# Rose-STL-Lab/dyffusion

Hardware: AMD Instinct MI355X
Metric: sampled fields/sec (h-step rollout) (higher is better)
Workload: dtype bf16; 1 GPU; BASELINE configs[1]: Navier-Stokes 221x42, C=3+2 static ch, unet_simple dim 64 @256^2, DYffusion h=16 cold sampling + refine, interpolator MC dropout p=0.15, hipGraph rollout; rows_per_gpu=80, total_rows=80, net_forwards_per_rollout=60, parallelism=ensemble-sharded dp1

## Files before the change

dyffusion_amd/csrc/engine.hip:

```cpp
#include "engine_internal.h"

#include <dlfcn.h>
#include <mutex>
#include <rccl/rccl.h>
#include "unet_kernels.h"
#include "../../include/dyffusion_hip_testing.h"

using namespace dyf;

namespace {

thread_local bool g_creating_group_child = false;

int default_row_groups(const dyf_engine* e) {
    if (e->cfg.net[0].arch != DYF_ARCH_UNET_RESNET || e->cfg.net[1].arch != DYF_ARCH_UNET_RESNET) return 1;
    if (e->cfg.batch_invariant) return 1;
    const long long plane = (long long)e->cfg.height * e->cfg.width;
    if (plane > 128 * 128) return 1;
    const long long pix = plane * e->cfg.max_batch;
    if (pix >= 72ll * 60 * 60) return 3;
    return 1;
}

void layout_blocks(Net& n) {
// ... 217 lines not shown
        if (f.up_cols) sparse_out = &b;
        const bool prof = e->prof_layer == i && e->prof_ev.size() < 4096;
        hipEvent_t pe0 = nullptr, pe1 = nullptr;
        if (prof) {
            HIP_TRY(e, hipEventCreate(&pe0));
            HIP_TRY(e, hipEventCreate(&pe1));
        }
        const bool commute = dyf_form_int("DYF_DEC_COMMUTE", 1) != 0;
        const bool commuted = commute && b.k == 1 && b.stride == 1 && b.pad == 0 && e->cfg.enable_mfma && (b.cout & 3) == 0 &&
                              (size_t)nb * lh * lw * b.cout * sizeof(float) <= (size_t)nb * b.in_h * b.in_w * b.cin * sizeof(el16_t);
        if (use_fused_up(e, b, f)) {
            if (prof) HIP_TRY(e, hipEventRecord(pe0, st));
            HIP_TRY(e, launch_conv(f, b.wpk, 1, st));
            if (prof) HIP_TRY(e, hipEventRecord(pe1, st));
        } else if (commuted) {
            ConvArgs lo = a;
            lo.src0 = x; lo.c0 = b.cin - skip_c; lo.src1 = skip; lo.c1 = skip_c;
            lo.h = lh; lo.w = lw; lo.ho = lh; lo.wo = lw;
            lo.coef_a = ws.ones_f; lo.coef_c = ws.zeros_f; lo.coef_stride = 0; lo.coef_div = 0;
            lo.act = ACT_NONE; lo.drop = DropSpec{};
            lo.out_el16 = nullptr; lo.out_f32 = (float*)ws.up;
            if (prof) HIP_TRY(e, hipEventRecord(pe0, st));
            dyf_status s = run_conv(e, lo, b.wpk, st);
            if (s != DYF_OK) return s;
            Up2xEpiArgs u{};
            u.lo = (const float*)ws.up; u.n = nb; u.h = lh; u.w = lw; u.c = b.cout;
            u.coef_a = a.coef_a; u.coef_c = a.coef_c; u.coef_stride = a.coef_stride; u.coef_div = a.coef_div;
            u.act = a.act; u.drop = a.drop; u.out = a.out_el16;
            HIP_TRY(e, launch_up2x_epilogue(u, st));
            if (prof) HIP_TRY(e, hipEventRecord(pe1, st));
        } else {
            Up2xArgs u{};
            u.src0 = x; u.c0 = b.cin - skip_c; u.src1 = skip; u.c1 = skip_c; u.n = nb; u.h = lh; u.w = lw; u.out = ws.up;
            HIP_TRY(e, launch_up2x(u, st));
            a.src0 = ws.up; a.c0 = b.cin; a.src1 = nullptr; a.c1 = 0;
            if (prof) HIP_TRY(e, hipEventRecord(pe0, st));
            dyf_status s = run_conv(e, a, b.wpk, st);
            if (s != DYF_OK) return s;
            if (prof) HIP_TRY(e, hipEventRecord(pe1, st));
        }
        if (prof) {
            e->prof_ev.emplace_back(pe0, pe1);
            e->prof_rows.push_back(nb);
        }
        x = ws.dec[i - 6];
        lh = b.out_h; lw = b.out_w;
        if (i < 11) {
            skip = ws.enc[10 - i];
            skip_c = n.blk[10 - i].cout;
        }
    }
    ReadoutArgs r{};
    r.x = x; r.n = nb; r.ih = lh; r.iw = lw; r.cin = n.dim; r.wgt = n.ro_w; r.wfrag = n.ro_wfrag; r.bias = n.ro_b; r.cout = n.cfg.out_channels;
    r.oh = H; r.ow = W; r.out = out_dev; r.nearest = n.cfg.outer_nearest;
    e->last_dec5_sparse = sparse_out != nullptr;
    r.iw_store = sparse_out ? sparse_out->up_wo_store : lw;
    r.col_map = sparse_out ? sparse_out->up_col_map : nullptr;
    if (n.ro_row_tab && (sparse_out != nullptr) == n.ro_tab_sparse) {
        r.row_tab = n.ro_row_tab;
        r.col_tab = n.ro_col_tab;
    }
    HIP_TRY(e, launch_readout(r, st));
    return DYF_OK;
}

dyf_status compute_coefs(dyf_engine* e, Net& n, const float* time_dev, int rows, float* coef_a, float* coef_c,
                         hipStream_t st) {
    FilmArgs f{};
    if (n.cfg.with_time_emb) {
        TimeMlpArgs t{};
        t.time = time_dev; t.rows = rows; t.dim = n.dim; t.w1 = n.t_w1; t.b1 = n.t_b1; t.w2 = n.t_w2; t.b2 = n.t_b2;
        t.silu_out = e->ws.silu;
        if (n.t_learned) { t.learned_w = n.t_learned; t.learned_half = n.cfg.learned_sinusoidal_dim / 2; }
        HIP_TRY(e, launch_time_mlp(t, st));
        f.silu = e->ws.silu;
    }
    f.rows = rows; f.tdim = n.tdim; f.total_c = n.total_c; f.wf = n.film_w; f.bf = n.film_b; f.blk_of = n.blk_of;
    f.blk_off = n.blk_off; f.blk_cout = n.blk_cout; f.norm_a = n.norm_a; f.norm_c = n.norm_c; f.coef_a = coef_a;
    f.coef_c = coef_c;
    HIP_TRY(e, launch_film(f, st));
    return DYF_OK;
}

}

extern "C" {

int32_t dyf_abi_version(void) { return DYF_ABI_VERSION; }

int32_t dyf_dtype(void) { return DYF_F16 ? DYF_DTYPE_F16 : DYF_DTYPE_BF16; }

const char* dyf_last_error(const dyf_engine* engine) { return engine ? engine->err.c_str() : g_create_error.c_str(); }

static void destroy_groups(dyf_engine* e) {
    for (dyf_engine* c : e->groups) {
        if (c->group_stream) { (void)hipStreamSynchronize(c->group_stream); (void)hipStreamDestroy(c->group_stream); }
        if (c->group_done) (void)hipEventDestroy(c->group_done);
        dyf_engine_destroy(c);
    }
    e->groups.clear();
    e->last_groups = 0;
}

static void traj_release(dyf_engine* e);

void dyf_engine_destroy(dyf_engine* e) {
    if (!e) return;
    (void)hipSetDevice(e->cfg.device);
    destroy_groups(e);
    if (e->group_fork) (void)hipEventDestroy(e->group_fork);
    for (auto& kv : e->graphs) {
        if (kv.second.exec) (void)hipGraphExecDestroy(kv.second.exec);
        if (kv.second.graph) (void)hipGraphDestroy(kv.second.graph);
    }
    rn_destroy(e->net[0]);
    rn_destroy(e->net[1]);
    sc_destroy(e->net[0]);
    sc_destroy(e->net[1]);
    (void)dyf_comm_destroy(e);
    if (e->s_log) (void)hipFree(e->s_log);
    if (e->cap_stream) (void)hipStreamDestroy(e->cap_stream);
    if (e->gn_err_host) (void)hipHostFree(e->gn_err_host);
    traj_release(e);
    f32_destroy(e);
    train_destroy(e);
    release_allocs(e->allocs);
    release_allocs(e->net_allocs[0]);
    release_allocs(e->net_allocs[1]);
    release_allocs(e->plan_allocs);
    delete e;
}

dyf_status dyf_engine_create(const dyf_engine_config* cfg, dyf_engine** out_engine) {
    if (!cfg || !out_engine) return fail(nullptr, DYF_ERR_INVALID_ARGUMENT, "null argument");
    if (cfg->abi_version != DYF_ABI_VERSION) return fail(nullptr, DYF_ERR_INVALID_ARGUMENT, "ABI version mismatch");
    if (cfg->dtype != dyf_dtype())
        return fail(nullptr, DYF_ERR_INVALID_ARGUMENT, std::string("this library is the ") + DYF_DTYPE_NAME +
                    " build: engine dtype must match (libdyffusion_hip.so = bf16, libdyffusion_hip_f16.so = fp16)");
    if (cfg->height < 1 || cfg->width < 1 || cfg->max_batch < 1)
        return fail(nullptr, DYF_ERR_INVALID_ARGUMENT, "height, width and max_batch must be positive");
    int ndev = 0;
    if (hipGetDeviceCount(&ndev) != hipSuccess || ndev < 1)
        return fail(nullptr, DYF_ERR_HIP, "no HIP device available: the DYffusion engine requires an MI355X (gfx950)");
    if (cfg->device < 0 || cfg->device >= ndev) return fail(nullptr, DYF_ERR_INVALID_ARGUMENT, "device ordinal out of range");
    if (hipSetDevice(cfg->device) != hipSuccess) return fail(nullptr, DYF_ERR_HIP, "hipSetDevice failed");

    dyf_engine* e = new dyf_engine();
    e->cfg = *cfg;
    e->fuse_up2x = dyf_form_int("DYF_FUSE_UP2X", e->fuse_up2x) != 0;
    e->fuse_min_plane = (int)dyf_form_int("DYF_FUSE_MIN_PLANE", e->fuse_min_plane);
    e->fuse_stem = dyf_form_int("DYF_FUSE_STEM", e->fuse_stem) != 0;
    e->pair_interp = dyf_form_int("DYF_PAIR_INTERP", e->pair_interp) != 0;
    e->poison_dec5 = dyf_form_int("DYF_POISON_DEC5", e->poison_dec5) != 0;
    if (conv_init() != hipSuccess || linattn_fused_init() != hipSuccess || hipStreamCreateWithFlags(&e->cap_stream, hipStreamNonBlocking) != hipSuccess) {
        delete e;
        return fail(nullptr, DYF_ERR_HIP, "engine initialisation failed (conv_init / stream create)");
    }
    auto bail = [&](dyf_status st, const std::string& m) {
        g_create_error = m;
        dyf_engine_destroy(e);
        return st;
    };
    for (int w = 0; w < 2; ++w) {
        Net& n = e->net[w];
        n.cfg = cfg->net[w];
        if (n.cfg.arch != DYF_ARCH_UNET_SIMPLE && n.cfg.arch != DYF_ARCH_UNET_RESNET && n.cfg.arch != DYF_ARCH_SIMPLE_CONV_NET)
            return bail(DYF_ERR_UNSUPPORTED, "arch must be unet_simple (0), unet / resnet (1) or simple_conv_net (2)");
        if (n.cfg.dim < 4 || (n.cfg.dim & 1)) return bail(DYF_ERR_INVALID_ARGUMENT, "dim must be even and >= 4");
        if (n.cfg.input_dropout < 0.0f || n.cfg.input_dropout >= 1.0f) return bail(DYF_ERR_INVALID_ARGUMENT, "input_dropout must be in [0, 1)");
        if (n.cfg.input_dropout != 0.0f && n.cfg.arch == DYF_ARCH_SIMPLE_CONV_NET)
            return bail(DYF_ERR_UNSUPPORTED, "input_dropout > 0: arch simple_conv_net has no such layer");
        if (n.cfg.dropout < 0.0f || n.cfg.dropout >= 1.0f) return bail(DYF_ERR_INVALID_ARGUMENT, "dropout must be in [0, 1)");
        n.cin_total = n.cfg.in_channels + n.cfg.cond_channels;
        if (n.cin_total < 1 || n.cin_total > DYF_MAX_IN_CH || n.cfg.out_channels < 1 || n.cfg.out_channels > DYF_MAX_OUT_CH)
            return bail(DYF_ERR_UNSUPPORTED, "channel counts outside the supported range (inputs+cond <= 32, outputs <= 8)");
        n.dim = n.cfg.dim;
        n.tdim = 2 * n.cfg.dim;
        if (n.cfg.arch == DYF_ARCH_UNET_RESNET) {
            if (n.cfg.block_dropout1 < 0.0f || n.cfg.block_dropout1 >= 1.0f || n.cfg.attn_dropout < 0.0f || n.cfg.attn_dropout >= 1.0f)
                return bail(DYF_ERR_INVALID_ARGUMENT, "dropout rates must be in [0, 1)");
            std::string m = rn_configure(e, n);
            if (!m.empty()) return bail(DYF_ERR_INVALID_ARGUMENT, m);
            continue;
        }
        if (n.cfg.arch == DYF_ARCH_SIMPLE_CONV_NET) {
            std::string m = sc_configure(e, n);
            if (!m.empty()) return bail(DYF_ERR_INVALID_ARGUMENT, m);
            continue;
        }
        n.n_drop_sites = (n.cfg.dropout > 0.0f ? 12 : 0) + (n.cfg.input_dropout > 0.0f ? 1 : 0);
        layout_blocks(n);
        std::string m = layout_geometry(n, cfg->height, cfg->width);
        if (!m.empty()) return bail(DYF_ERR_INVALID_ARGUMENT, m);
    }
    const size_t nb = (size_t)cfg->max_batch * 2;
    size_t stem_el = 0, enc_el[6] = {}, dec_el[6] = {}, up_el = 0, raw_el = 0, tc = 0, td = 0, ub_el = 0;
    for (int w = 0; w < 2; ++w) {
        const Net& n = e->net[w];
        stem_el = std::max(stem_el, nb * n.uh * n.uw * n.dim);
        for (int i = 0; i < 6; ++i) {
            const UBlock& b = n.blk[i];
            enc_el[i] = std::max(enc_el[i], nb * b.out_h * b.out_w * b.cout);
            const UBlock& d = n.blk[6 + i];
            dec_el[i] = std::max(dec_el[i], nb * d.out_h * d.out_w * d.cout);
            up_el = std::max(up_el, nb * d.in_h * d.in_w * d.cin);
            ub_el = std::max(ub_el, conv_up_border_floats((int)nb, d.out_h / 2, d.out_w / 2, d.cout));
        }
        raw_el = std::max(raw_el, nb * n.blk[5].out_h * n.blk[5].out_w * n.blk[5].cout);
        tc = std::max<size_t>(tc, n.total_c);
        td = std::max<size_t>(td, n.tdim);
    }
    Workspace& ws = e->ws;
#define ALLOC(ptr, count)                                           \
    do {                                                            \
        dyf_status _s = dev_alloc(e, &(ptr), (count));              \
        if (_s != DYF_OK) return bail(_s, e->err);                  \
    } while (0)
    ALLOC(ws.stem, stem_el);
    {
        size_t s16 = 0;
        for (int w = 0; w < 2; ++w) s16 = std::max(s16, nb * (size_t)(e->net[w].uh + 2) * (e->net[w].uw + 2) * 16);
        ALLOC(ws.stem16, s16);
    }
    for (int i = 0; i < 6; ++i) {
        ALLOC(ws.enc[i], enc_el[i]);
        ALLOC(ws.dec[i], dec_el[i]);
    }
    ALLOC(ws.enc5_raw, raw_el);
    ALLOC(ws.up, up_el);
    ALLOC(ws.silu, nb * td);
    ALLOC(ws.coef_a, nb * tc);
    ALLOC(ws.coef_c, nb * tc);
    ALLOC(ws.zero_page, 256);
    ALLOC(ws.up_border, ub_el);
    ALLOC(ws.coef_pair, 4 * tc);
    ALLOC(ws.splitk, DYF_SPLITK_FLOATS);
    {
        size_t cmax = 64;
        for (int w = 0; w < 2; ++w)
            for (int i = 0; i < 12; ++i) cmax = std::max<size_t>(cmax, (size_t)e->net[w].blk[i].cout);
        ALLOC(ws.zeros_f, cmax);
        ALLOC(ws.ones_f, cmax);
        std::vector<float> ones(cmax, 1.0f);
        if (hipMemcpy(ws.ones_f, ones.data(), cmax * sizeof(float), hipMemcpyHostToDevice) != hipSuccess)
            return bail(DYF_ERR_HIP, "hipMemcpy(ones)");
    }
    ALLOC(e->s_pair, 2 * (size_t)cfg->max_batch * DYF_MAX_OUT_CH * cfg->height * cfg->width);
    ALLOC(e->s_time, 64);
    ALLOC(e->rng_state, DYF_RNG_STATE_WORDS);
    ALLOC(e->row_keys, 4 * nb);
#undef ALLOC
    if (hipHostMalloc((void**)&e->gn_err_host, 64, hipHostMallocMapped) == hipSuccess) {
        memset(e->gn_err_host, 0, 64);
        if (hipHostGetDevicePointer((void**)&e->gn_err_dev, e->gn_err_host, 0) != hipSuccess) e->gn_err_dev = nullptr;
    }
    if (!e->gn_err_dev) e->gn_fuse_disabled = true;
    if (dyf_form_int("DYF_GN_FUSED", 1) == 0) e->gn_fuse_disabled = true;
    {
        dyf_status rs = rn_alloc_workspace(e);
        if (rs != DYF_OK) return bail(rs, e->err);
        rs = sc_alloc_workspace(e);
        if (rs != DYF_OK) return bail(rs, e->err);
    }
    e->group_min_rows = (int)std::max(1LL, dyf_form_int("DYF_GROUP_MIN_ROWS", e->group_min_rows));
    *out_engine = e;
    if (!g_creating_group_child) {
        const int g = (int)dyf_form_int("DYF_ROW_GROUPS", default_row_groups(e));
        if (g > 1) {
            dyf_status gs = dyf_set_row_groups(e, g);
            if (gs != DYF_OK) {
                g_create_error = e->err;
                dyf_engine_destroy(e);
                *out_engine = nullptr;
                return gs;
            }
        }
    }
    return DYF_OK;
}

dyf_status dyf_set_row_groups(dyf_engine* e, int32_t n_groups) {
    if (!e) return DYF_ERR_INVALID_ARGUMENT;
    if (e->is_group_child) return fail(e, DYF_ERR_STATE, "row groups do not nest");
    if (n_groups < 1 || n_groups > 8) return fail(e, DYF_ERR_INVALID_ARGUMENT, "n_groups must be in [1, 8]");
    if (e->net[0].loaded || e->net[1].loaded)
        return fail(e, DYF_ERR_STATE, "dyf_set_row_groups must be called before dyf_load_weights (the groups hold their own packed weights)");
    HIP_TRY(e, hipSetDevice(e->cfg.device));
    HIP_TRY(e, hipDeviceSynchronize());
    destroy_groups(e);
    if (n_groups == 1 || e->cfg.max_batch < 2 * e->group_min_rows) return DYF_OK;
    n_groups = std::min<int>(n_groups, e->cfg.max_batch / e->group_min_rows);
    if (!e->group_fork) HIP_TRY(e, hipEventCreateWithFlags(&e->group_fork, hipEventDisableTiming));
    dyf_engine_config cc = e->cfg;
    cc.max_batch = (e->cfg.max_batch + std::min(n_groups, 2) - 1) / std::min(n_groups, 2);
    for (int g = 0; g < n_groups; ++g) {
        dyf_engine* c = nullptr;
        g_creating_group_child = true;
        dyf_status cs = dyf_engine_create(&cc, &c);
        g_creating_group_child = false;
        if (cs != DYF_OK) {
            destroy_groups(e);
            return fail(e, cs, "row group engine: " + g_create_error);
        }
        c->is_group_child = true;
        c->attn_dropout_exact = e->attn_dropout_exact;
        c->form_rows_scale = dyf_form_int("DYF_GROUP_FORM_SCALE", 1) != 0 ? n_groups : 1;
        e->groups.push_back(c);
// ... 1943 lines not shown
```

dyffusion_amd/csrc/kernels.h:

```cpp
#pragma once
#include "common.h"

#include <vector>

#define DYF_MAX_IN_CH 32
#define DYF_MAX_OUT_CH 8

struct TimeMlpArgs {
    const float* time;
    int rows, dim;
    const float* w1;
    const float* b1;
    const float* w2;
    const float* b2;
    float* silu_out;
    const float* learned_w = nullptr;
    int learned_half = 0;
};
hipError_t launch_time_mlp(const TimeMlpArgs& a, hipStream_t s);

struct FilmArgs {
    const float* silu;
    int rows, tdim, total_c;
    const float* wf;
    const float* bf;
    const int* blk_of;
    const int* blk_off;
    const int* blk_cout;
    const float* norm_a;
    const float* norm_c;
    float* coef_a;
    float* coef_c;
};
hipError_t launch_film(const FilmArgs& a, hipStream_t s);

struct StemArgs {
    const float* src[4];
    int ch[4];
    int nsrc, cin;
    int n, h, w;
    int src_rows;
    int out_pitch;
    int distinct_only;
    int uh, uw;
    int resample;
    int nearest;
    const float* wgt;
    const float* bias;
    int dim;
    el16_t* out;
    DropSpec drop;
    uint32_t* rng_state;
    uint32_t* rng_row_keys;
    int rng_rows, rng_rows_per_fwd;
};
hipError_t launch_stem(const StemArgs& a, hipStream_t s);
hipError_t launch_stem16(const StemArgs& a, hipStream_t s);
inline __host__ __device__ int stem16_out_rows(const StemArgs& a) { return a.distinct_only && a.src_rows > 0 ? a.src_rows : a.n; }

struct Up2xArgs {
    const el16_t* src0;
    const el16_t* src1;
    int c0, c1;
    int n, h, w;
    el16_t* out;
};
hipError_t launch_up2x(const Up2xArgs& a, hipStream_t s);

struct Up2xEpiArgs {
    const float* lo;
    int n, h, w, c;
    const float* coef_a;
    const float* coef_c;
    int coef_stride, coef_div;
    int act;
    DropSpec drop;
    el16_t* out;
};
hipError_t launch_up2x_epilogue(const Up2xEpiArgs& a, hipStream_t s);

struct GroupNormArgs {
    const float* x;
    int n, hw, c, groups;
    const float* gamma;
    const float* beta;
    const float* film_a;
    const float* film_c;
    int film_stride;
    int film_div;
    int act;
    DropSpec drop;
    el16_t* out;
};
hipError_t launch_groupnorm(const GroupNormArgs& a, hipStream_t s);

struct ReadoutArgs {
    const el16_t* x;
    int n, ih, iw, cin;
    int iw_store;
    const int16_t* col_map;
    const float* wgt;
    const el16_t* wfrag;
    const float* bias;
    int cout;
    int oh, ow;
    int nearest;
    float* out;
    const uint4* row_tab;
    const uint4* col_tab;
};
hipError_t launch_readout(const ReadoutArgs& a, hipStream_t s);
hipError_t launch_readout_tables(const ReadoutArgs& a, hipStream_t s);
inline std::vector<float> pack_readout_weights(const float* w, int cin, int cout) {
    std::vector<float> pk((size_t)16 * cin * cout);
    for (int ci = 0; ci < cin; ++ci)
        for (int co = 0; co < cout; ++co)
            for (int t = 0; t < 16; ++t) pk[((size_t)t * cin + ci) * cout + co] = w[((size_t)ci * cout + co) * 16 + t];
    return pk;
}
inline std::vector<el16_t> pack_readout_frag(const std::vector<float>& pk, int cout) {
    std::vector<el16_t> wf((size_t)16 * 2 * 64 * 8, 0);
    for (int t = 0; t < 16; ++t)
        for (int h2 = 0; h2 < 2; ++h2)
            for (int lane = 0; lane < 64; ++lane) {
                const int m = lane & 15, kg = lane >> 4;
                for (int el = 0; el < 8; ++el)
                    if (m < cout)
                        wf[(((size_t)t * 2 + h2) * 64 + lane) * 8 + el] = f32_to_el16(pk[((size_t)t * 64 + h2 * 32 + kg * 8 + el) * cout + m]);
            }
    return wf;
}

hipError_t launch_cold_update(float* x_s, const float* x_cur, const float* x_next, long long count, hipStream_t s, float* copy = nullptr);
hipError_t launch_noisy_condition(float* out, const float* cond, const float* noise, float tau, long long count,
                                  int row_elems, uint32_t* rng_state, hipStream_t s);
#define DYF_RNG_STATE_WORDS 8

struct BcArgs {
    float* preds;
    int kind;
    int n_fields, rows, c, h, w, n_meta;
    const int* row_meta;
    const float* time_factor;
    int times_per_meta;
    const uint8_t* fixed_mask;
    const float* in_velocity;
    const float* vertex_y;
    const float* boundary;
};
hipError_t launch_boundary_conditions(const BcArgs& a, hipStream_t s);
hipError_t launch_nhwc_to_nchw_f32(const el16_t* src, int n, int h, int w, int w_store, int c, const int16_t* col_map,
                                   float* out, hipStream_t s);
hipError_t launch_rng_clone(uint32_t* dst, const uint32_t* src, uint32_t row_add, bool counters_only, hipStream_t s);
hipError_t launch_rng_begin_forward(uint32_t* rng_state, uint32_t* row_keys, int rows, int rows_per_fwd, hipStream_t s);
hipError_t launch_fill_f32(float* p, float v, long long count, hipStream_t s);
hipError_t launch_criterion_sum(const float* p, const float* t, long long count, int kind, double* sum, hipStream_t s);
constexpr int CRITERION_MAX_BLOCKS = 2048;
hipError_t launch_criterion_sum_det(const float* p, const float* t, long long count, int kind, double* partials, double* sum, hipStream_t s);
hipError_t launch_ensemble_metrics(const float* preds, const float* targets, int n_members, long long n_points, double* sums,
                                   hipStream_t s);
long long trajectory_metrics_blocks(int n_members, long long n_points);
hipError_t launch_trajectory_metrics(const float* const* preds_tab, const float* const* targets_tab, int n_segments, int n_members,
                                     long long n_points, long long member_stride, double* partials, double* out, double* accum,
                                     hipStream_t s);

hipError_t launch_gather_unpack(const float* recv, float* out, int world, int slots, int nb, int total_rows, long long row, hipStream_t s);
```

dyffusion_amd/csrc/kernels.hip:

```cpp
#include "kernels.h"

#include <cstdlib>

__device__ __forceinline__ float wave_sum(float v) {
#pragma unroll
    for (int off = 32; off > 0; off >>= 1) v += __shfl_xor(v, off, 64);
    return v;
}

__device__ __forceinline__ float block_sum(float v, float* scratch ) {
    v = wave_sum(v);
    const int lane = threadIdx.x & 63, wave = threadIdx.x >> 6, nw = (blockDim.x + 63) >> 6;
    __syncthreads();
    if (lane == 0) scratch[wave] = v;
    __syncthreads();
    float t = 0.0f;
    for (int i = 0; i < nw; ++i) t += scratch[i];
    return t;
}

__global__ void time_mlp_kernel(TimeMlpArgs a) {
    extern __shared__ float sh[];
    const int row = blockIdx.x, tdim = 2 * a.dim, half = a.dim / 2;
    const int dim = a.learned_w ? 2 * a.learned_half + 1 : a.dim;
// ... 1002 lines not shown
    }
#endif
}

__global__ void readout_tables_kernel(ReadoutArgs a, uint4* row_tab, uint4* col_tab) {
    const int t = blockIdx.x * blockDim.x + threadIdx.x;
    const int th = 2 * a.ih, tw = 2 * a.iw;
    if (t < a.oh) {
        int u0, u1;
        float lu;
        bilinear_coord(t, (float)th / (float)a.oh, th, u0, u1, lu, a.nearest != 0);
        int off[4];
        float w[4];
        for (int k = 0; k < 4; ++k) {
            const int par = (k + 1) & 1;
            w[k] = ((u0 & 1) == par ? 1.0f - lu : 0.0f) + ((u1 & 1) == par ? lu : 0.0f);
            const int u = (u1 & 1) == par ? u1 : u0;
            const int i = ((u + 1) >> 1) - (k >> 1);
            off[k] = (unsigned)i < (unsigned)a.ih ? i * a.iw_store * 128 : -1;
        }
        row_tab[2 * t] = make_uint4((unsigned)off[0], (unsigned)off[1], (unsigned)off[2], (unsigned)off[3]);
        row_tab[2 * t + 1] = make_uint4(__float_as_uint(w[0]), __float_as_uint(w[1]), __float_as_uint(w[2]), __float_as_uint(w[3]));
    }
    if (t < a.ow) {
        int v0, v1;
        float lv;
        bilinear_coord(t, (float)tw / (float)a.ow, tw, v0, v1, lv, a.nearest != 0);
        int off[4];
        float w[4];
        for (int k = 0; k < 4; ++k) {
            const int par = (k + 1) & 1;
            w[k] = ((v0 & 1) == par ? 1.0f - lv : 0.0f) + ((v1 & 1) == par ? lv : 0.0f);
            const int v = (v1 & 1) == par ? v1 : v0;
            const int j = ((v + 1) >> 1) - (k >> 1);
            int js = (unsigned)j < (unsigned)a.iw ? j : -1;
            if (js >= 0 && a.col_map) js = a.col_map[js];
            off[k] = js >= 0 ? js * 128 : -1;
        }
        col_tab[2 * t] = make_uint4((unsigned)off[0], (unsigned)off[1], (unsigned)off[2], (unsigned)off[3]);
        col_tab[2 * t + 1] = make_uint4(__float_as_uint(w[0]), __float_as_uint(w[1]), __float_as_uint(w[2]), __float_as_uint(w[3]));
    }
}

hipError_t launch_readout_tables(const ReadoutArgs& a, hipStream_t s) {
    const int n = a.oh > a.ow ? a.oh : a.ow;
    hipLaunchKernelGGL(readout_tables_kernel, dim3((n + 255) / 256), dim3(256), 0, s, a, (uint4*)a.row_tab, (uint4*)a.col_tab);
    return hipGetLastError();
}

__global__ __launch_bounds__(256, 4) void readout_dma_kernel(ReadoutArgs a, int groups_per_wave) {
#if defined(__HIP_DEVICE_COMPILE__)
    extern __shared__ __attribute__((aligned(16))) char rd_smem[];
    for (int i = threadIdx.x; i < 16 * 2 * 4 * 4; i += 256) {
        const int m = i & 3, kg = (i >> 2) & 3, th = i >> 4;
        ((uint4*)rd_smem)[i] = ((const uint4*)a.wfrag)[th * 64 + kg * 16 + m];
    }
    __syncthreads();
    const int lane = threadIdx.x & 63, wave = threadIdx.x >> 6;
    const int wave_id = (int)((blockIdx.x * 256 + threadIdx.x) >> 6);
    const int p = lane & 15, kg = lane >> 4;
    char* stage = rd_smem + 8192 + wave * 8192;
    const uint4* wl = (const uint4*)rd_smem + kg * 4 + (p & 3);
    const bool wrow = p < 4;
    const int total = a.n * a.oh * a.ow;
    const int th = 2 * a.ih, tw = 2 * a.iw;
    const float sh = (float)th / (float)a.oh, sw = (float)tw / (float)a.ow;
    const int plane = a.oh * a.ow;
    const size_t xbytes = (size_t)a.n * a.ih * a.iw_store * 64 * sizeof(el16_t);
    const auto rsrc = __builtin_amdgcn_make_buffer_rsrc((void*)a.x, 0, (int)(unsigned)xbytes, 0x00020000);
    const int lp = lane >> 2, lc = lane & 3;
    const unsigned piece_off = (unsigned)((lc ^ (lp & 3)) * 16);
    const int src4 = lp * 4;
    const unsigned rd_off = (unsigned)((p * 4 + (kg ^ (p & 3))) * 16);
    for (int g = 0; g < groups_per_wave; ++g) {
        const int idx0 = (wave_id * groups_per_wave + g) * 16;
        if (idx0 >= total) break;
        int idx = idx0 + p;
        const bool live = idx < total;
        if (!live) idx = total - 1;
        const int n = idx / plane;
        const int rem = idx - n * plane;
        const int oy = rem / a.ow, ox = rem - oy * a.ow;
        const uint4 rto = a.row_tab[2 * oy], rtw = a.row_tab[2 * oy + 1], cto = a.col_tab[2 * ox], ctw = a.col_tab[2 * ox + 1];
        const int nbase = n * a.ih * a.iw_store * 128;
        const int rto_[4] = {(int)rto.x, (int)rto.y, (int)rto.z, (int)rto.w};
        const int ro[4] = {rto_[0] >= 0 ? nbase + rto_[0] : -1, rto_[1] >= 0 ? nbase + rto_[1] : -1, rto_[2] >= 0 ? nbase + rto_[2] : -1,
                           rto_[3] >= 0 ? nbase + rto_[3] : -1};
        const int co_[4] = {(int)cto.x, (int)cto.y, (int)cto.z, (int)cto.w};
        const float rw[4] = {__uint_as_float(rtw.x), __uint_as_float(rtw.y), __uint_as_float(rtw.z), __uint_as_float(rtw.w)};
        const float cw[4] = {__uint_as_float(ctw.x), __uint_as_float(ctw.y), __uint_as_float(ctw.z), __uint_as_float(ctw.w)};
        int l_ro[4], l_co[4];
#pragma unroll
        for (int k = 0; k < 4; ++k) {
            l_ro[k] = __builtin_amdgcn_ds_bpermute(src4, ro[k]);
            l_co[k] = __builtin_amdgcn_ds_bpermute(src4, co_[k]);
        }
        float out[4] = {0.0f, 0.0f, 0.0f, 0.0f};
        auto issue = [&](int bt) {
            const int kh = bt >> 1;
            char* st = stage + (bt & 1) * 4096;
#pragma unroll
            for (int t = 0; t < 2; ++t) {
                const int kw = (bt & 1) * 2 + t;
                const bool ok = l_ro[kh] >= 0 && l_co[kw] >= 0;
                const unsigned vo = ok ? (unsigned)(l_ro[kh] + l_co[kw]) + piece_off : 0xFFFFFFFFu;
                __builtin_amdgcn_raw_ptr_buffer_load_lds(rsrc, (__attribute__((address_space(3))) void*)(st + (t * 2 + 0) * 1024), 16, vo, 0, 0, 0);
                __builtin_amdgcn_raw_ptr_buffer_load_lds(rsrc, (__attribute__((address_space(3))) void*)(st + (t * 2 + 1) * 1024), 16,
                                                         ok ? vo + 64u : 0xFFFFFFFFu, 0, 0, 0);
            }
        };
        asm volatile("s_waitcnt lgkmcnt(0)" ::: "memory");
        issue(0);
#pragma unroll
        for (int bt = 0; bt < 8; ++bt) {
            if (bt + 1 < 8) {
                asm volatile("s_waitcnt lgkmcnt(0)" ::: "memory");
                issue(bt + 1);
                asm volatile("s_waitcnt vmcnt(4)" ::: "memory");
            } else {
                asm volatile("s_waitcnt vmcnt(0)" ::: "memory");
            }
            const int kh = bt >> 1;
            const char* st = stage + (bt & 1) * 4096;
#pragma unroll
            for (int t = 0; t < 2; ++t) {
                const int kw = (bt & 1) * 2 + t, tap = kh * 4 + kw;
                const uint4 b0 = *(const uint4*)(st + (t * 2 + 0) * 1024 + rd_off);
                const uint4 b1 = *(const uint4*)(st + (t * 2 + 1) * 1024 + rd_off);
                uint4 w0 = make_uint4(0u, 0u, 0u, 0u), w1 = w0;
                if (wrow) {
                    w0 = wl[(tap * 2 + 0) * 16];
                    w1 = wl[(tap * 2 + 1) * 16];
                }
                ro_f32x4 d = {0.0f, 0.0f, 0.0f, 0.0f};
                d = DYF_MFMA_16x16x32(__builtin_bit_cast(el16x8_t, w0), __builtin_bit_cast(el16x8_t, b0), d, 0, 0, 0);
                d = DYF_MFMA_16x16x32(__builtin_bit_cast(el16x8_t, w1), __builtin_bit_cast(el16x8_t, b1), d, 0, 0, 0);
                const float bw = (ro[kh] >= 0 && co_[kw] >= 0) ? rw[kh] * cw[kw] : 0.0f;
#pragma unroll
                for (int r = 0; r < 4; ++r) out[r] = fmaf(bw, d[r], out[r]);
            }
        }
        if (live && kg == 0) {
            float* o = a.out + ((size_t)n * a.cout * a.oh + oy) * a.ow + ox;
            const size_t cs = (size_t)a.oh * a.ow;
            o[0] = out[0] + a.bias[0];
            if (a.cout > 1) o[cs] = out[1] + a.bias[1];
            if (a.cout > 2) o[2 * cs] = out[2] + a.bias[2];
            if (a.cout > 3) o[3 * cs] = out[3] + a.bias[3];
        }
    }
#endif
}

hipError_t launch_readout(const ReadoutArgs& a, hipStream_t s) {
    const long long total = (long long)a.n * a.oh * a.ow;
    const bool regw = dyf_form_int("DYF_READOUT_REGW", 1) != 0;
    const bool use_mfma = dyf_form_int("DYF_READOUT_MFMA", 1) != 0;
    if (a.col_map && !(a.wfrag && a.cin == 64 && a.cout >= 1 && a.cout <= 4)) return hipErrorInvalidValue;
    if ((use_mfma || a.col_map) && a.wfrag && a.cin == 64 && a.cout >= 1 && a.cout <= 4 && total < (1ll << 30)) {
        const long long groups = (total + 15) / 16;
        long long waves = 256ll * 16;
        int per = (int)((groups + waves - 1) / waves);
        if (per < 1) per = 1;
        waves = (groups + per - 1) / per;
        const bool use_dma = dyf_form_int("DYF_READOUT_DMA", 1) != 0;
        const bool dma = use_dma && a.row_tab && a.col_tab && (size_t)a.n * a.ih * a.iw_store * 128 < 0x7F000000ull;
        dyf_form_note(dma ? "readout_dma_kernel" : "readout_mfma_kernel", a.n);
        KernelProf kp(dma ? "readout_dma_kernel" : "readout_mfma_kernel", s,
                      (double)a.n * a.ih * a.iw_store * a.cin * 2.0 + (double)a.n * a.cout * a.oh * a.ow * 4.0);
        if (dma)
            hipLaunchKernelGGL(readout_dma_kernel, dim3((unsigned)((waves + 3) / 4)), dim3(256), 8192 + 4 * 8192, s, a, per);
        else
            hipLaunchKernelGGL(readout_mfma_kernel, dim3((unsigned)((waves + 3) / 4)), dim3(256), 32768, s, a, per);
        return hipGetLastError();
    }
    if (regw && a.cin == 64 && a.cout >= 1 && a.cout <= 4 && total < (1ll << 30)) {
        int halves = 256 * 16 * 2;
        int per = (int)((total + halves - 1) / halves);
        if (per < 8) per = 8;
        per += per & 1;
        halves = (int)((total + per - 1) / per);
        const unsigned blocks = (unsigned)((halves + 7) / 8);
#define RW_CASE(C)                                                                                      \
        if (a.cout == C) {                                                                              \
            dyf_form_note("readout_regw_kernel<" #C ">", a.n);                                          \
            hipLaunchKernelGGL(readout_regw_kernel<C>, dim3(blocks), dim3(256), 0, s, a, per);          \
            return hipGetLastError();                                                                   \
        }
        RW_CASE(1) RW_CASE(2) RW_CASE(3) RW_CASE(4)
#undef RW_CASE
    }
    const size_t lds = (size_t)16 * a.cin * a.cout * sizeof(float);
    const int lanes = (a.cin % 8 == 0) ? a.cin / 8 : 0;
#define RO_CASE(L)                                                                                                   \
    if (lanes == L) {                                                                                                \
        dyf_form_note("readout_sliced_kernel<" #L ">", a.n);                                                         \
        hipLaunchKernelGGL(readout_sliced_kernel<L>, dim3((unsigned)((total * L + 255) / 256)), dim3(256), lds, s, a); \
        return hipGetLastError();                                                                                    \
    }
    RO_CASE(1) RO_CASE(2) RO_CASE(4) RO_CASE(8) RO_CASE(16)
#undef RO_CASE
    dyf_form_note("readout_kernel", a.n);
    hipLaunchKernelGGL(readout_kernel, dim3((unsigned)((total + 255) / 256)), dim3(256), lds, s, a);
    return hipGetLastError();
}

__global__ void cold_update_kernel(float* x_s, const float* x_cur, const float* x_next, long long count, float* copy) {
    const long long i = (long long)blockIdx.x * blockDim.x + threadIdx.x;
    if (i < count) {
        const float v = x_s[i] - x_cur[i] + x_next[i];
        x_s[i] = v;
        if (copy) copy[i] = v;
    }
}

hipError_t launch_cold_update(float* x_s, const float* x_cur, const float* x_next, long long count, hipStream_t s, float* copy) {
    hipLaunchKernelGGL(cold_update_kernel, dim3((unsigned)((count + 255) / 256)), dim3(256), 0, s, x_s, x_cur, x_next,
                       count, copy);
    return hipGetLastError();
}

__global__ void noisy_condition_kernel(float* out, const float* cond, const float* noise, float tau, long long count,
                                       int row_elems, const uint32_t* rng_state) {
    const long long i = (long long)blockIdx.x * blockDim.x + threadIdx.x;
    if (i >= count) return;
    float z;
    if (noise != nullptr) {
        z = noise[i];
    } else {
        const uint32_t n = (uint32_t)(i / row_elems), e = (uint32_t)(i - (long long)n * row_elems);
        const RngKey rk = rng_row_key(rng_state[0], rng_state[1] ^ 0x4E6F6973u, rng_state[4], rng_state[3] + n);
        const uint32_t w0 = fmix32(e * 0x9E3779B1u + rk.k0), w1 = fmix32(w0 ^ rk.k1);
        const float u1 = ((float)(w0 >> 8) + 0.5f) * (1.0f / 16777216.0f);
        const float u2 = ((float)(w1 >> 8) + 0.5f) * (1.0f / 16777216.0f);
        z = sqrtf(-2.0f * logf(u1)) * cosf(6.283185307179586f * u2);
    }
    out[i] = tau * cond[i] + (1.0f - tau) * z;
}

__global__ void rng_bump_kernel(uint32_t* state, int slot, uint32_t by) {
    if (threadIdx.x == 0 && blockIdx.x == 0) state[slot] += by;
}

__global__ void rng_clone_kernel(uint32_t* dst, const uint32_t* src, uint32_t row_add, int counters_only) {
    if (threadIdx.x != 0 || blockIdx.x != 0) return;
    if (counters_only) {
        dst[2] = src[2];
        dst[4] = src[4];
        return;
    }
    for (int i = 0; i < DYF_RNG_STATE_WORDS; ++i) dst[i] = src[i];
    dst[3] = src[3] + row_add;
}

hipError_t launch_rng_clone(uint32_t* dst, const uint32_t* src, uint32_t row_add, bool counters_only, hipStream_t s) {
    hipLaunchKernelGGL(rng_clone_kernel, dim3(1), dim3(64), 0, s, dst, src, row_add, counters_only ? 1 : 0);
    return hipGetLastError();
}

hipError_t launch_noisy_condition(float* out, const float* cond, const float* noise, float tau, long long count,
                                  int row_elems, uint32_t* rng_state, hipStream_t s) {
    hipLaunchKernelGGL(noisy_condition_kernel, dim3((unsigned)((count + 255) / 256)), dim3(256), 0, s, out, cond, noise,
                       tau, count, row_elems, rng_state);
    if (noise == nullptr)
        hipLaunchKernelGGL(rng_bump_kernel, dim3(1), dim3(64), 0, s, rng_state, 4, 1u);
    return hipGetLastError();
}

__global__ __launch_bounds__(256) void rng_begin_forward_kernel(uint32_t* state, uint32_t* row_keys, int rows, int rows_per_fwd) {
    const uint32_t lo = state[0], hi = state[1], fwd0 = state[2], row0 = state[3];
    for (int r = threadIdx.x; r < rows; r += blockDim.x) {
        const RngKey k = rng_row_key(lo, hi, fwd0 + (uint32_t)(r / rows_per_fwd), row0 + (uint32_t)(r % rows_per_fwd));
        row_keys[2 * r] = k.k0;
        row_keys[2 * r + 1] = k.k1;
    }
    __syncthreads();
    if (threadIdx.x == 0) state[2] = fwd0 + (uint32_t)((rows + rows_per_fwd - 1) / rows_per_fwd);
}

hipError_t launch_rng_begin_forward(uint32_t* rng_state, uint32_t* row_keys, int rows, int rows_per_fwd, hipStream_t s) {
    hipLaunchKernelGGL(rng_begin_forward_kernel, dim3(1), dim3(256), 0, s, rng_state, row_keys, rows, rows_per_fwd);
    return hipGetLastError();
}

__global__ void boundary_conditions_kernel(BcArgs a) {
    const long long i = (long long)blockIdx.x * blockDim.x + threadIdx.x;
    const int chw = a.c * a.h * a.w;
    const long long total = (long long)a.n_fields * a.rows * chw;
    if (i >= total) return;
    const int e = (int)(i % chw);
    const int row = (int)((i / chw) % a.rows), f = (int)(i / ((long long)chw * a.rows));
    const int b = a.row_meta[row];
    if (b < 0) return;
    const bool fixed = a.fixed_mask[(size_t)b * chw + e] != 0;
    if (a.kind == 0) {
        if (e < a.w) {
            const float growth = a.time_factor[a.times_per_meta ? f * a.n_meta + b : f];
            const float vy = a.vertex_y[(size_t)b * a.w + e];
            const float s0 = (float)((double)a.in_velocity[b] * 4.0);
            float v = s0 * vy;
            v = v * (0.41f - vy);
            v = v / (float)(0.41 * 0.41);
            a.preds[i] = v * growth;
        } else if (fixed) {
            a.preds[i] = 0.0f;
        }
    } else if (fixed) {
        a.preds[i] = a.boundary[(size_t)b * chw + e];
    }
}

hipError_t launch_boundary_conditions(const BcArgs& a, hipStream_t s) {
    const long long total = (long long)a.n_fields * a.rows * a.c * a.h * a.w;
    hipLaunchKernelGGL(boundary_conditions_kernel, dim3((unsigned)((total + 255) / 256)), dim3(256), 0, s, a);
    return hipGetLastError();
}

__global__ void nhwc_to_nchw_f32_kernel(const el16_t* src, int n, int h, int w, int w_store, int c, const int16_t* col_map,
                                        float* out) {
    const long long i = (long long)blockIdx.x * blockDim.x + threadIdx.x;
    const long long total = (long long)n * c * h * w;
    if (i >= total) return;
    const int x = (int)(i % w), y = (int)((i / w) % h), ch = (int)((i / ((long long)w * h)) % c), b = (int)(i / ((long long)w * h * c));
// ... 436 lines not shown
```

Measured before the change: 9190 fields/s.

## Add row-banded DMA readout kernel that reuses staged input rows across output bands

Adds a new readout kernel in which each workgroup handles a band of output rows for one sample. Input rows stream into LDS through buffer-load-to-LDS with a triple-buffered pipeline. Each staged row is projected once via MFMA into per-tap partials, which are then bilinearly combined for every output pixel in the band. The aim is to stop re-gathering overlapping input rows for each output pixel group. The cost is a larger LDS footprint (up to 80 KB, requiring a function attribute set at init) and a band-size heuristic, so fewer workgroups may be resident.

After: 9334 fields/s (median of 6 runs). +1.6%, better.

```diff
diff --git a/dyffusion_amd/csrc/engine.hip b/dyffusion_amd/csrc/engine.hip
--- a/dyffusion_amd/csrc/engine.hip
+++ b/dyffusion_amd/csrc/engine.hip
@@ -393,7 +393,7 @@
     e->fuse_stem = dyf_form_int("DYF_FUSE_STEM", e->fuse_stem) != 0;
     e->pair_interp = dyf_form_int("DYF_PAIR_INTERP", e->pair_interp) != 0;
     e->poison_dec5 = dyf_form_int("DYF_POISON_DEC5", e->poison_dec5) != 0;
-    if (conv_init() != hipSuccess || linattn_fused_init() != hipSuccess || hipStreamCreateWithFlags(&e->cap_stream, hipStreamNonBlocking) != hipSuccess) {
+    if (conv_init() != hipSuccess || linattn_fused_init() != hipSuccess || readout_init() != hipSuccess || hipStreamCreateWithFlags(&e->cap_stream, hipStreamNonBlocking) != hipSuccess) {
         delete e;
         return fail(nullptr, DYF_ERR_HIP, "engine initialisation failed (conv_init / stream create)");
     }
diff --git a/dyffusion_amd/csrc/kernels.h b/dyffusion_amd/csrc/kernels.h
--- a/dyffusion_amd/csrc/kernels.h
+++ b/dyffusion_amd/csrc/kernels.h
@@ -110,6 +110,7 @@
     const uint4* col_tab;
 };
 hipError_t launch_readout(const ReadoutArgs& a, hipStream_t s);
+hipError_t readout_init();
 hipError_t launch_readout_tables(const ReadoutArgs& a, hipStream_t s);
 inline std::vector<float> pack_readout_weights(const float* w, int cin, int cout) {
     std::vector<float> pk((size_t)16 * cin * cout);
diff --git a/dyffusion_amd/csrc/kernels.hip b/dyffusion_amd/csrc/kernels.hip
--- a/dyffusion_amd/csrc/kernels.hip
+++ b/dyffusion_amd/csrc/kernels.hip
@@ -1178,6 +1178,196 @@
 #endif
 }
 
+#define RR_MAXQ 4
+#define RR_NOCOL 0xFFFFFFFFu
+#define RR_BARRIER() asm volatile("s_waitcnt lgkmcnt(0)\n\ts_barrier" ::: "memory")
+typedef __attribute__((ext_vector_type(4))) unsigned ro_u32x4;
+__device__ __forceinline__ void rr_read_frags(unsigned a0, unsigned a1, unsigned b0, unsigned b1, ro_u32x4& x0, ro_u32x4& x1, ro_u32x4& y0, ro_u32x4& y1) {
+    asm volatile("ds_read_b128 %0, %4\n\tds_read_b128 %1, %5\n\tds_read_b128 %2, %6\n\tds_read_b128 %3, %7\n\ts_waitcnt lgkmcnt(0)"
+                 : "=&v"(x0), "=&v"(x1), "=&v"(y0), "=&v"(y1) : "v"(a0), "v"(a1), "v"(b0), "v"(b1) : "memory");
+}
+__device__ __forceinline__ void rr_read_z4(unsigned a0, unsigned a1, unsigned a2, unsigned a3, ro_f32x4& z0, ro_f32x4& z1, ro_f32x4& z2, ro_f32x4& z3) {
+    asm volatile("ds_read_b128 %0, %4\n\tds_read_b128 %1, %5\n\tds_read_b128 %2, %6\n\tds_read_b128 %3, %7\n\ts_waitcnt lgkmcnt(0)"
+                 : "=&v"(z0), "=&v"(z1), "=&v"(z2), "=&v"(z3) : "v"(a0), "v"(a1), "v"(a2), "v"(a3) : "memory");
+}
+__device__ __forceinline__ void rr_write_z(unsigned addr, ro_f32x4 d) { asm volatile("ds_write_b128 %0, %1" : : "v"(addr), "v"(d) : "memory"); }
+
+__global__ __launch_bounds__(256) void readout_dma_rows_kernel(ReadoutArgs a, int band, int nbands, int G) {
+#if defined(__HIP_DEVICE_COMPILE__)
+    extern __shared__ __attribute__((aligned(16))) char rr_smem[];
+    const int tid = threadIdx.x, lane = tid & 63, wave = tid >> 6;
+    const int p = lane & 15, kg = lane >> 4;
+    const int n = (int)blockIdx.x / nbands, oy0 = ((int)blockIdx.x - n * nbands) * band;
+    const int rows_here = (a.oh - oy0 < band ? a.oh - oy0 : band);
+    const int rowbytes = a.iw_store * 128, WC = G * 16;
+    const unsigned z0 = (unsigned)(size_t)(__attribute__((address_space(3))) char*)rr_smem;
+    const unsigned stage0 = z0 + (unsigned)(G * 4096);
+    char* stage = rr_smem + G * 4096;
+    const int stage_sz = G * 2048;
+    const int tiles = (a.iw_store + 7) / 8;
+    const int ntile = wave < tiles ? (tiles - wave + 3) / 4 : 0;
+    uint4 A[4][2];
+#pragma unroll
+    for (int kh = 0; kh < 4; ++kh)
+#pragma unroll
+        for (int h = 0; h < 2; ++h) A[kh][h] = ((const uint4*)a.wfrag)[((kh * 4 + (p >> 2)) * 2 + h) * 64 + kg * 16 + (p & 3)];
+    int rhi = -1, rlo = 0x7FFFFFFF;
+    if (lane < rows_here) {
+        const uint4 o = a.row_tab[2 * (oy0 + lane)];
+        const int ov[4] = {(int)o.x, (int)o.y, (int)o.z, (int)o.w};
+#pragma unroll
+        for (int k = 0; k < 4; ++k)
+            if (ov[k] >= 0) {
+                rhi = ov[k] > rhi ? ov[k] : rhi;
+                rlo = ov[k] < rlo ? ov[k] : rlo;
+            }
+    }
+#pragma unroll
+    for (int off = 32; off > 0; off >>= 1) {
+        const int h2 = __shfl_xor(rhi, off, 64), l2 = __shfl_xor(rlo, off, 64);
+        rhi = h2 > rhi ? h2 : rhi;
+        rlo = l2 < rlo ? l2 : rlo;
+    }
+    rhi = __builtin_amdgcn_readfirstlane(rhi);
+    rlo = __builtin_amdgcn_readfirstlane(rlo);
+    int ro[RR_MAXQ][4];
+    unsigned zc[RR_MAXQ][4];
+    float rw[RR_MAXQ][4], cw[RR_MAXQ][4], out[RR_MAXQ][4];
+    const int npix = rows_here * a.ow;
+#pragma unroll
+    for (int q = 0; q < RR_MAXQ; ++q) {
+        const int pix = tid + 256 * q;
+        const bool ok = pix < npix;
+        const int oyl = ok ? pix / a.ow : 0, ox = ok ? pix - oyl * a.ow : 0;
+        const uint4 rto = a.row_tab[2 * (oy0 + oyl)], rtw = a.row_tab[2 * (oy0 + oyl) + 1];
+        const uint4 cto = a.col_tab[2 * ox], ctw = a.col_tab[2 * ox + 1];
+        ro[q][0] = ok ? (int)rto.x : -2; ro[q][1] = ok ? (int)rto.y : -2; ro[q][2] = ok ? (int)rto.z : -2; ro[q][3] = ok ? (int)rto.w : -2;
+        zc[q][0] = (int)cto.x >= 0 ? cto.x >> 3 : RR_NOCOL; zc[q][1] = (int)cto.y >= 0 ? cto.y >> 3 : RR_NOCOL;
+        zc[q][2] = (int)cto.z >= 0 ? cto.z >> 3 : RR_NOCOL; zc[q][3] = (int)cto.w >= 0 ? cto.w >> 3 : RR_NOCOL;
+        rw[q][0] = __uint_as_float(rtw.x); rw[q][1] = __uint_as_float(rtw.y); rw[q][2] = __uint_as_float(rtw.z); rw[q][3] = __uint_as_float(rtw.w);
+        cw[q][0] = __uint_as_float(ctw.x); cw[q][1] = __uint_as_float(ctw.y); cw[q][2] = __uint_as_float(ctw.z); cw[q][3] = __uint_as_float(ctw.w);
+#pragma unroll
+        for (int c = 0; c < 4; ++c) out[q][c] = 0.0f;
+    }
+    const size_t xbytes = (size_t)a.n * a.ih * a.iw_store * 64 * sizeof(el16_t);
+    const auto rsrc = __builtin_amdgcn_make_buffer_rsrc((void*)a.x, 0, (int)(unsigned)xbytes, 0x00020000);
+    const unsigned nbase = (unsigned)n * (unsigned)a.ih * (unsigned)rowbytes;
+    const int lp = lane >> 3;
+    const unsigned piece_off = (unsigned)(((lane & 7) ^ lp) * 16);
+    const unsigned rd_base = (unsigned)((p >> 3) * 1024 + (p & 7) * 128);
+    const unsigned rd_off0 = rd_base + (unsigned)((kg ^ (p & 7)) * 16), rd_off1 = rd_base + (unsigned)(((4 + kg) ^ (p & 7)) * 16);
+    const unsigned zw = z0 + (unsigned)((kg * WC + p) * 16);
+    auto issue = [&](int rb, int b) {
+        for (int t = 0; t < ntile; ++t) {
+            const int tile = wave + 4 * t, px = tile * 8 + lp;
+            const bool ok = rb >= rlo && px < a.iw_store;
+            const unsigned vo = ok ? nbase + (unsigned)rb + (unsigned)(px * 128) + piece_off : 0xFFFFFFFFu;
+            __builtin_amdgcn_raw_ptr_buffer_load_lds(rsrc, (__attribute__((address_space(3))) void*)(stage + b * stage_sz + tile * 1024), 16, vo, 0, 0, 0);
+        }
+    };
+    if (rhi >= 0) {
+        issue(rhi, 0);
+        issue(rhi - rowbytes, 1);
+        int b = 0;
+        for (int rb = rhi; rb >= rlo; rb -= rowbytes) {
+            switch (ntile) {
+                case 0: break;
+                case 1: asm volatile("s_waitcnt vmcnt(1)" ::: "memory"); break;
+                case 2: asm volatile("s_waitcnt vmcnt(2)" ::: "memory"); break;
+                case 3: asm volatile("s_waitcnt vmcnt(3)" ::: "memory"); break;
+                default: asm volatile("s_waitcnt vmcnt(4)" ::: "memory"); break;
+            }
+            RR_BARRIER();
+            issue(rb - 2 * rowbytes, b == 0 ? 2 : b - 1);
+            if (wave < G) {
+                const bool two = wave + 4 < G;
+                const unsigned st = stage0 + (unsigned)(b * stage_sz + wave * 2048), st2 = st + (two ? 4 * 2048u : 0u);
+                ro_u32x4 x0, x1, y0, y1;
+                rr_read_frags(st + rd_off0, st + rd_off1, st2 + rd_off0, st2 + rd_off1, x0, x1, y0, y1);
+#pragma unroll
+                for (int kh = 0; kh < 4; ++kh) {
+                    ro_f32x4 d = {0.0f, 0.0f, 0.0f, 0.0f};
+                    d = DYF_MFMA_16x16x32(__builtin_bit_cast(el16x8_t, A[kh][0]), __builtin_bit_cast(el16x8_t, x0), d, 0, 0, 0);
+                    d = DYF_MFMA_16x16x32(__builtin_bit_cast(el16x8_t, A[kh][1]), __builtin_bit_cast(el16x8_t, x1), d, 0, 0, 0);
+                    rr_write_z(zw + (unsigned)(kh * 4 * WC * 16 + wave * 256), d);
+                }
+                if (two) {
+#pragma unroll
+                    for (int kh = 0; kh < 4; ++kh) {
+                        ro_f32x4 d = {0.0f, 0.0f, 0.0f, 0.0f};
+                        d = DYF_MFMA_16x16x32(__builtin_bit_cast(el16x8_t, A[kh][0]), __builtin_bit_cast(el16x8_t, y0), d, 0, 0, 0);
+                        d = DYF_MFMA_16x16x32(__builtin_bit_cast(el16x8_t, A[kh][1]), __builtin_bit_cast(el16x8_t, y1), d, 0, 0, 0);
+                        rr_write_z(zw + (unsigned)(kh * 4 * WC * 16 + (wave + 4) * 256), d);
+                    }
+                }
+            }
+            RR_BARRIER();
+#pragma unroll
+            for (int q = 0; q < RR_MAXQ; ++q)
+#pragma unroll
+                for (int kh = 0; kh < 4; ++kh)
+                    if (ro[q][kh] == rb) {
+                        ro_f32x4 zv[4];
+                        const unsigned zr = z0 + (unsigned)(kh * 4 * WC * 16);
+                        rr_read_z4(zr + (zc[q][0] != RR_NOCOL ? zc[q][0] : 0u), zr + (unsigned)(WC * 16) + (zc[q][1] != RR_NOCOL ? zc[q][1] : 0u),
+                                   zr + (unsigned)(2 * WC * 16) + (zc[q][2] != RR_NOCOL ? zc[q][2] : 0u),
+                                   zr + (unsigned)(3 * WC * 16) + (zc[q][3] != RR_NOCOL ? zc[q][3] : 0u), zv[0], zv[1], zv[2], zv[3]);
+#pragma unroll
+                        for (int kw = 0; kw < 4; ++kw) {
+                            const bool ok = zc[q][kw] != RR_NOCOL;
+                            const float bw = ok ? rw[q][kh] * cw[q][kw] : 0.0f;
+#pragma unroll
+                            for (int c = 0; c < 4; ++c) out[q][c] = fmaf(bw, ok ? zv[kw][c] : 0.0f, out[q][c]);
+                        }
+                    }
+            b = b == 2 ? 0 : b + 1;
+        }
+    }
+    const size_t cs = (size_t)a.oh * a.ow;
+#pragma unroll
+    for (int q = 0; q < RR_MAXQ; ++q) {
+        const int pix = tid + 256 * q;
+        if (pix < npix) {
+            if (ro[q][3] == -1) {
+#pragma unroll
+                for (int c = 0; c < 4; ++c) out[q][c] = fmaf(0.0f, 0.0f, out[q][c]);
+            }
+            float* o = a.out + ((size_t)n * a.cout * a.oh + oy0) * a.ow + pix;
+            o[0] = out[q][0] + a.bias[0];
+            if (a.cout > 1) o[cs] = out[q][1] + a.bias[1];
+            if (a.cout > 2) o[2 * cs] = out[q][2] + a.bias[2];
+            if (a.cout > 3) o[3 * cs] = out[q][3] + a.bias[3];
+        }
+    }
+#endif
+}
+
+static size_t readout_rows_lds(int iw_store, int* G) {
+    *G = (iw_store + 15) / 16;
+    return (size_t)*G * 4096 + (size_t)3 * *G * 2048;
+}
+static int readout_rows_band(const ReadoutArgs& a) {
+    int cap = RR_MAXQ * 256 / a.ow;
+    cap = cap > 64 ? 64 : cap;
+    cap = cap > a.oh ? a.oh : cap;
+    int best = cap;
+    double best_cost = 0.0;
+    for (int band = cap; band >= (cap < 8 ? cap : 8); --band) {
+        const long long wgs = (long long)a.n * ((a.oh + band - 1) / band);
+        const double cost = (double)((wgs + 511) / 512) * ((double)band * a.ih / a.oh + 3.0);
+        if (band == cap || cost < best_cost) {
+            best = band;
+            best_cost = cost;
+        }
+    }
+    return best;
+}
+#define RR_LDS_MAX (80 * 1024)
+
+hipError_t readout_init() {
+    return hipFuncSetAttribute((const void*)readout_dma_rows_kernel, hipFuncAttributeMaxDynamicSharedMemorySize, RR_LDS_MAX);
+}
+
 hipError_t launch_readout(const ReadoutArgs& a, hipStream_t s) {
     const long long total = (long long)a.n * a.oh * a.ow;
     const bool regw = dyf_form_int("DYF_READOUT_REGW", 1) != 0;
@@ -1194,7 +1384,14 @@
         dyf_form_note(dma ? "readout_dma_kernel" : "readout_mfma_kernel", a.n);
         KernelProf kp(dma ? "readout_dma_kernel" : "readout_mfma_kernel", s,
                       (double)a.n * a.ih * a.iw_store * a.cin * 2.0 + (double)a.n * a.cout * a.oh * a.ow * 4.0);
-        if (dma)
+        int G = 0;
+        const size_t rows_lds = readout_rows_lds(a.iw_store, &G);
+        const bool rows = dma && dyf_form_int("DYF_READOUT_ROWS", 1) != 0 && rows_lds <= RR_LDS_MAX && a.ow <= RR_MAXQ * 256;
+        if (dma) dyf_form_note(rows ? "readout_dma_kernel+rows" : "readout_dma_kernel+gather", a.n);
+        if (rows) {
+            const int band = readout_rows_band(a), nbands = (a.oh + band - 1) / band;
+            hipLaunchKernelGGL(readout_dma_rows_kernel, dim3((unsigned)(a.n * nbands)), dim3(256), rows_lds, s, a, band, nbands, G);
+        } else if (dma)
             hipLaunchKernelGGL(readout_dma_kernel, dim3((unsigned)((waves + 3) / 4)), dim3(256), 8192 + 4 * 8192, s, a, per);
         else
             hipLaunchKernelGGL(readout_mfma_kernel, dim3((unsigned)((waves + 3) / 4)), dim3(256), 32768, s, a, per);
```
